# vinhsuhi/JMAC

Hardware: AMD Instinct MI355X
Metric: gnn_layer_edges_per_s (higher is better)
Workload: dtype f32

## Files before the change

include/jmac_hip.h:

```cpp
#ifndef JMAC_HIP_H_
#define JMAC_HIP_H_

#include <stddef.h>
#include <stdint.h>

#ifdef __cplusplus
extern "C" {
#endif

typedef void* jmac_stream_t;

#define JMAC_OK 0
#define JMAC_EINVAL (-1)
#define JMAC_EDIM (-2)
#define JMAC_EWORKSPACE (-3)
#define JMAC_ERANGE (-4)

typedef struct { int32_t seg, beg, end, pslot; } jmac_item_t;
typedef struct { int32_t seg, pslot0, nchunks, pad; } jmac_split_t;

const char* jmac_strerror(int rc);
int jmac_version(void);


// ... 233 lines not shown
} jmac_gemm_task_t;
int jmac_gemm_grouped_f32(const jmac_gemm_task_t* tasks, int32_t n_tasks, jmac_stream_t stream);

#define JMAC_WCAT_MAX 4
int jmac_wcat_pack_seed_f32(const float* const* w_att, const float* const* gcn, float* const* wcat, int32_t n_layers,
                            int64_t d, const float* extra_src, float* extra_dst, int64_t extra_floats,
                            int64_t* const* counters, int32_t n_counters, int64_t* seed_state, int64_t* seed_out,
                            jmac_stream_t stream);
int jmac_wcat_unpack_f32(const float* const* dwcat, float* const* d_watt, float* const* d_gcn,
                         int32_t n_layers, int64_t d, const float* extra_src, float* extra_dst,
                         int64_t extra_floats, jmac_stream_t stream);

#define JMAC_ADAM_MAX_TASKS 64
typedef struct {
    float* p;
    const float* g;
    float* m;
    float* v;
    int64_t n;
    int32_t vec4;
} jmac_adam_task_t;
int jmac_adam_step_f32(const jmac_adam_task_t* tasks, int32_t n_tasks, float* step, double* aux, double lr, double beta1,
                       double beta2, double eps, double weight_decay, int32_t decoupled, int32_t maximize, jmac_stream_t stream);

int jmac_rows_compact_f32(const float* const* h_src, const int64_t* h_ld_src, float* const* h_dst, int32_t n_tables,
                          const int64_t* idx, int64_t n_used, int64_t d, jmac_stream_t stream);
int jmac_rows_expand_f32(const float* const* h_src, float* const* h_dst, const int64_t* h_ld_dst,
                         const int32_t* h_accumulate, int32_t n_tables, const int32_t* pos, int64_t rows, int64_t d,
                         jmac_stream_t stream);


int jmac_triple_l1_fwd_f32(const float* ent, int64_t lde, const float* rel, int64_t ldr,
                           const int64_t* h, const int64_t* r, const int64_t* t, int64_t T,
                           int64_t period, int64_t d, float* score, jmac_stream_t stream);
int jmac_triple_l1_bwd_f32(const float* ent, int64_t lde, const float* rel, int64_t ldr,
                           const int64_t* h, const int64_t* r, const int64_t* t, int64_t T,
                           int64_t period, int64_t d, const float* gscore, float* dent, int64_t ldde, float* drel, int64_t lddr,
                           jmac_stream_t stream);
int jmac_pair_cosine_fwd_stats_f32(const float* e1, int64_t ld1, const float* e2, int64_t ld2, const int64_t* i1,
                                   const int64_t* i2, int64_t L, int64_t d, float* dist, float* stats,
                                   jmac_stream_t stream);
int jmac_pair_cosine_bwd_rows_f32(const float* e1, int64_t ld1, const float* e2, int64_t ld2, int64_t L, int64_t d,
                                  const float* gdist, const float* gscalar, float gscale, const float* stats,
                                  const int32_t* rec, const int32_t* rowptr, int64_t n1, int64_t n2, float* de1,
                                  int64_t ldd1, float* de2, int64_t ldd2, jmac_stream_t stream);

int jmac_triple_l1_margin_bwd_exact2_f32(const float* ent, int64_t lde, const float* rel, int64_t ldr, const int64_t* h,
                                         const int64_t* r, const int64_t* t, int64_t B, int64_t K, int64_t d,
                                         const float* score, const float* gamma, const float* gloss, int64_t ent_off,
                                         int64_t rel_off, float* cnt_ent, float* cnt_rel, float* dent, int64_t rows_ent,
                                         int32_t acc_ent, float* drel, int64_t rows_rel, int32_t acc_rel,
                                         jmac_stream_t stream);

int jmac_vec_mean_acc_f32(const float* x, int64_t n, const float* add_to, float* out, jmac_stream_t stream);

int jmac_pair_cosine_fwd_f32(const float* e1, int64_t ld1, const float* e2, int64_t ld2,
                             const int64_t* i1, const int64_t* i2, int64_t L, int64_t d, float* dist,
                             jmac_stream_t stream);
int jmac_pair_cosine_bwd_f32(const float* e1, int64_t ld1, const float* e2, int64_t ld2,
                             const int64_t* i1, const int64_t* i2, int64_t L, int64_t d,
                             const float* gdist, float* de1, int64_t ldd1, float* de2, int64_t ldd2,
                             jmac_stream_t stream);

int jmac_margin_loss_fwd_acc_f32(const float* score, int64_t B, int64_t K, const float* gamma, const float* add_to,
                                 float* loss, jmac_stream_t stream);
int jmac_margin_loss_bwd_f32(const float* score, int64_t B, int64_t K, const float* gamma,
                             const float* gloss, float* dscore, jmac_stream_t stream);


int jmac_sample_completion_batch(const int64_t* triples, int64_t T, const int64_t* perm, const int32_t* key_of_triple,
                                 const int32_t* tail_ptr, const int32_t* tail_idx, int64_t num_ent, int64_t B, int64_t K,
                                 const int64_t* seed, int64_t* step, int64_t* batch_h, int64_t* batch_r, int64_t* batch_t,
                                 jmac_stream_t stream);

int jmac_scatter_sum_f32(const float* src, const int64_t* index, int64_t E, int64_t d, int64_t N,
                         float* out, jmac_stream_t stream);
size_t jmac_scatter_softmax_workspace_bytes(int64_t N, int64_t d);
int jmac_scatter_softmax_f32(const float* src, const int64_t* index, int64_t E, int64_t d, int64_t N,
                             float* out, void* ws, size_t ws_bytes, jmac_stream_t stream);

#ifdef __cplusplus
}
#endif
#endif
```

jmac_amd/_lib.py:

```python
from __future__ import annotations

import ctypes as C
import os
import re
import weakref
from typing import Optional

_HERE = os.path.dirname(os.path.abspath(__file__))
LIB_PATH = os.environ.get("JMAC_LIB_PATH") or os.path.join(_HERE, "libjmac_hip.so")
HEADER_PATH = os.path.join(os.path.dirname(_HERE), "include", "jmac_hip.h")

_lib: Optional[C.CDLL] = None

i32, i64, f32, vp, sz = C.c_int32, C.c_int64, C.c_float, C.c_void_p, C.c_size_t


class JmacError(RuntimeError):
    pass


class View(C.Structure):
    _fields_ = [("ptr", vp), ("order", vp), ("items", vp), ("splits", vp), ("counts", vp),
                ("n_items_max", i64), ("n_splits_max", i64), ("n_parts_max", i64),
                ("item_edges", vp), ("n_empty", i64), ("n_coop", i64), ("entry_dst", vp)]
# ... 55 lines not shown
                                        vp, sz, vp]),
    "jmac_bn_tanh_bwd2_f32": (C.c_int, [vp, i64, vp, i64, vp, i64, vp, i64, i64, i64, vp, vp, vp, i32, vp, i64, vp, vp,
                                        vp, sz, vp]),
    "jmac_bn_tanh_seg_workspace_bytes": (sz, [i32, i64]),
    "jmac_bn_tanh_seg_fwd2_f32": (C.c_int, [vp, i64, i64, i32, C.POINTER(i64), C.POINTER(i32), vp, vp, vp, vp, f32, f32, vp, i64,
                                            vp, i64, vp, vp, vp, sz, vp]),
    "jmac_bn_tanh_seg_bwd2_f32": (C.c_int, [vp, i64, vp, i64, vp, i64, vp, i64, i64, i32, C.POINTER(i64), vp, vp, vp, vp, i64,
                                            vp, vp, vp, sz, vp]),
    "jmac_row_normalize_drop_fwd_f32": (C.c_int, [vp, i64, i64, i64, f32, vp, i64, f32, vp, i64, vp, vp]),
    "jmac_row_normalize_drop_bwd_f32": (C.c_int, [vp, i64, vp, vp, i64, f32, vp, i64, i64, i64, f32, vp, i64, i32, vp]),
    "jmac_row_normalize_dropseed_fwd_f32": (C.c_int, [vp, i64, i64, i64, f32, vp, f32, vp, i64, vp, vp]),
    "jmac_row_normalize_dropseed_bwd_f32": (C.c_int, [vp, i64, vp, vp, f32, vp, i64, i64, i64, f32, vp, i64, i32, vp]),
    "jmac_gemm_grouped_f32": (C.c_int, [C.POINTER(GemmTask), i32, vp]),
    "jmac_wcat_pack_seed_f32": (C.c_int, [C.POINTER(vp), C.POINTER(vp), C.POINTER(vp), i32, i64, vp, vp, i64, C.POINTER(vp), i32, vp, vp, vp]),
    "jmac_adam_step_f32": (C.c_int, [C.POINTER(AdamTask), i32, vp, vp, C.c_double, C.c_double, C.c_double, C.c_double, C.c_double, i32, i32,
                                     vp]),
    "jmac_wcat_unpack_f32": (C.c_int, [C.POINTER(vp), C.POINTER(vp), C.POINTER(vp), i32, i64, vp, vp, i64, vp]),
    "jmac_rows_compact_f32": (C.c_int, [C.POINTER(vp), C.POINTER(i64), C.POINTER(vp), i32, vp, i64, i64, vp]),
    "jmac_rows_expand_f32": (C.c_int, [C.POINTER(vp), C.POINTER(vp), C.POINTER(i64), C.POINTER(i32), i32, vp, i64, i64, vp]),
    "jmac_col_moments_f32": (C.c_int, [vp, i64, i64, i64, vp, vp, vp, sz, vp]),
    "jmac_bn_tanh_apply_f32": (C.c_int, [vp, i64, i64, i64, vp, vp, vp, vp, vp, i64, vp]),
    "jmac_bn_tanh_bwd_sums_f32": (C.c_int, [vp, i64, vp, i64, vp, i64, i64, i64, vp, vp, vp, vp, sz, vp]),
    "jmac_bn_tanh_bwd_apply_f32": (C.c_int, [vp, i64, vp, i64, vp, i64, i64, i64, vp, vp, vp, vp, i64, vp, i64, vp]),
    "jmac_row_normalize_fwd_f32": (C.c_int, [vp, i64, i64, i64, f32, vp, i64, vp, vp]),
    "jmac_row_normalize_bwd_f32": (C.c_int, [vp, i64, vp, i64, vp, i64, i64, f32, vp, i64, vp]),
    "jmac_l1_score_f32": (C.c_int, [vp, i64, vp, i64, i64, i64, i64, vp, i64, i32, vp]),
    "jmac_l1_score_bf16": (C.c_int, [vp, i64, vp, i64, i64, i64, i64, vp, i64, i32, vp]),
    "jmac_filtered_rank_f32": (C.c_int, [vp, i64, vp, vp, vp, i64, i64, i32, vp, vp]),
    "jmac_linkpred_rank_workspace_bytes": (sz, [i64, i64, i32]),
    "jmac_linkpred_rank_f32": (C.c_int, [vp, i32, vp, vp, i32, vp, vp, vp, i64, i64, i64, vp, vp, sz, vp]),
    "jmac_linkpred_rank_bf16": (C.c_int, [vp, i32, vp, vp, i32, vp, vp, vp, i64, i64, i64, vp, vp, sz, vp]),
    "jmac_sim_matrix_f32": (C.c_int, [vp, i64, vp, i64, i64, i64, i64, vp, i64, vp]),
    "jmac_sim_topk_workspace_bytes": (sz, [i64, i64, i32]),
    "jmac_sim_topk_f32": (C.c_int, [vp, i64, vp, i64, i64, i64, i64, i32, vp, vp, vp, sz, vp]),
    "jmac_col_topk_workspace_bytes": (sz, [i64, i64, i32]),
    "jmac_col_topk_f32": (C.c_int, [vp, i64, i64, i64, i32, vp, vp, sz, vp]),
    "jmac_row_topk_f32": (C.c_int, [vp, i64, i64, i64, i32, vp, vp, vp]),
    "jmac_softmax_entropy_workspace_bytes": (sz, [i64, i64]),
    "jmac_softmax_entropy_f32": (C.c_int, [vp, i64, vp, i64, i64, i64, i64, f32, vp, vp, vp, sz, vp]),
    "jmac_row_softmax_f32": (C.c_int, [vp, i64, i64, i64, vp, vp, f32, f32, vp, i64, vp, vp]),
    "jmac_col_softmax_workspace_bytes": (sz, [i64, i64]),
    "jmac_col_softmax_f32": (C.c_int, [vp, i64, i64, i64, vp, vp, f32, f32, vp, i64, vp, vp, sz, vp]),
    "jmac_csls_rank_f32": (C.c_int, [vp, i64, i64, i64, vp, vp, vp, vp, vp]),
    "jmac_csls_apply_f32": (C.c_int, [vp, i64, i64, i64, vp, vp, vp, i64, vp]),
    "jmac_gemm_f32": (C.c_int, [vp, i64, i32, vp, i64, i32, i64, i64, i64, vp, i64, vp]),
    "jmac_triple_l1_fwd_f32": (C.c_int, [vp, i64, vp, i64, vp, vp, vp, i64, i64, i64, vp, vp]),
    "jmac_triple_l1_bwd_f32": (C.c_int, [vp, i64, vp, i64, vp, vp, vp, i64, i64, i64, vp, vp, i64, vp, i64, vp]),
    "jmac_pair_cosine_fwd_stats_f32": (C.c_int, [vp, i64, vp, i64, vp, vp, i64, i64, vp, vp, vp]),
    "jmac_pair_cosine_fwd_f32": (C.c_int, [vp, i64, vp, i64, vp, vp, i64, i64, vp, vp]),
    "jmac_pair_cosine_bwd_f32": (C.c_int, [vp, i64, vp, i64, vp, vp, i64, i64, vp, vp, i64, vp, i64, vp]),
    "jmac_pair_cosine_bwd_rows_f32": (C.c_int, [vp, i64, vp, i64, i64, i64, vp, vp, f32, vp, vp, vp, i64, i64, vp, i64, vp, i64, vp]),
    "jmac_triple_l1_margin_bwd_exact2_f32": (C.c_int, [vp, i64, vp, i64, vp, vp, vp, i64, i64, i64, vp, vp, vp, i64, i64, vp, vp,
                                                       vp, i64, i32, vp, i64, i32, vp]),
    "jmac_vec_mean_acc_f32": (C.c_int, [vp, i64, vp, vp, vp]),
    "jmac_margin_loss_fwd_acc_f32": (C.c_int, [vp, i64, i64, vp, vp, vp, vp]),
    "jmac_margin_loss_bwd_f32": (C.c_int, [vp, i64, i64, vp, vp, vp, vp]),
    "jmac_sample_completion_batch": (C.c_int, [vp, i64, vp, vp, vp, vp, i64, i64, i64, vp, vp, vp, vp, vp, vp]),
    "jmac_scatter_sum_f32": (C.c_int, [vp, vp, i64, i64, i64, vp, vp]),
    "jmac_scatter_softmax_workspace_bytes": (sz, [i64, i64]),
    "jmac_scatter_softmax_f32": (C.c_int, [vp, vp, i64, i64, i64, vp, vp, sz, vp]),
}


_TESTING_SIGS = {
    "jmac_gemm_nt_x3_f32": (C.c_int, [vp, i64, vp, i64, i64, i64, i64, vp, i64, vp]),
}


def header_text(path: str = HEADER_PATH) -> str:
    return re.sub(r"/\*.*?\*/", "", open(path).read(), flags=re.S)


def header_symbols(path: str = HEADER_PATH):
    return sorted(set(re.findall(r"\b(jmac_[a-z0-9_]+)\s*\(", header_text(path))))


def lib() -> C.CDLL:
    global _lib
    if _lib is None:
        if not os.path.exists(LIB_PATH):
            raise JmacError(
                "jmac_amd: %s is missing. Build it with `python -c \"import __graft_entry__ as g; g.build()\"` "
                "(or `make -C jmac_amd/csrc`). There is no CPU fallback." % LIB_PATH)
        import torch
        l = C.CDLL(LIB_PATH)
        for name, (res, args) in _SIGS.items():
            fn = getattr(l, name)
            fn.restype = res
            fn.argtypes = args
        _lib = l
    return _lib


_tlib: Optional[C.CDLL] = None


def testing_lib() -> C.CDLL:
    global _tlib
    if _tlib is None:
        path = os.path.join(_HERE, "libjmac_hip_testing.so")
        if not os.path.exists(path):
            raise JmacError("jmac_amd: %s is missing (the atomic backward lives in the testing build only: "
                            "`make -C jmac_amd/csrc`)" % path)
        import torch
        l = C.CDLL(path)
        for name in ("jmac_rel_attn_aggregate_bwd_f32", "jmac_rel_attn_bwd_workspace_bytes", "jmac_strerror"):
# ... 88 lines not shown
```

jmac_amd/csrc/loss.hip:

```cpp
#include "common.h"

using namespace jmac;

namespace {

constexpr int kBlock = 256;
constexpr int kWavesPerBlock = kBlock / 64;

__device__ __forceinline__ float sgn(float x) { return x > 0.f ? 1.f : (x < 0.f ? -1.f : 0.f); }

template <int NK>
__global__ __launch_bounds__(kBlock) void triple_l1_fwd_kernel(const float* __restrict__ ent, int64_t lde,
                                                               const float* __restrict__ rel, int64_t ldr,
                                                               const int64_t* __restrict__ h, const int64_t* __restrict__ r,
                                                               const int64_t* __restrict__ t, int64_t T, int64_t period, int parts,
                                                               int d, float* __restrict__ score) {
    const int lane = lane_id();
    const int64_t w0 = (int64_t)blockIdx.x * kWavesPerBlock + (threadIdx.x >> 6);
    const int64_t nw = (int64_t)gridDim.x * kWavesPerBlock;
    const int64_t nrun = (period < T ? period : T) * parts;
    const int64_t stride = period * parts;
    for (int64_t u = w0; u < nrun; u += nw) {
        const int64_t b = u / parts, p = u % parts;
        int64_t ch = -1, cr = -1;
// ... 95 lines not shown
                const int c = lane + 64 * k;
                if (c < d && acc[k] != 0.f) {
                    atomicAdd(qh + c, acc[k]);
                    atomicAdd(qr + c, acc[k]);
                }
            }
        };
        int64_t x = b + p * period;
        while (x < T) {
            const int64_t x2 = x + stride;
            const bool in2 = x2 < T;
            const int64_t ih = h[x], ir = r[x], it = t[x];
            const int64_t ih2 = h[in2 ? x2 : x], ir2 = r[in2 ? x2 : x], it2 = t[in2 ? x2 : x];
            const bool pair = in2 && ih2 == ih && ir2 == ir;
            if (ih != ch || ir != cr) {
                flush();
                ch = ih;
                cr = ir;
                const float* ph = ent + ih * lde;
                const float* pr = rel + ir * ldr;
#pragma unroll
                for (int k = 0; k < NK; ++k) {
                    const int c = lane + 64 * k;
                    hr[k] = c < d ? ph[c] + pr[c] : 0.f;
                    acc[k] = 0.f;
                }
            }
            const float g = gof(x), g2 = pair ? gof(x2) : 0.f;
            const float* pt = ent + it * lde;
            const float* pt2 = ent + (pair ? it2 : it) * lde;
            float* qt = dent + it * ldde;
            float* qt2 = dent + (pair ? it2 : it) * ldde;
            float tv[NK], tv2[NK];
#pragma unroll
            for (int k = 0; k < NK; ++k) {
                const int c = lane + 64 * k;
                tv[k] = c < d ? pt[c] : 0.f;
                tv2[k] = c < d ? pt2[c] : 0.f;
            }
#pragma unroll
            for (int k = 0; k < NK; ++k) {
                const int c = lane + 64 * k;
                if (c < d) {
                    const float v = g * sgn(hr[k] - tv[k]);
                    const float v2 = g2 * sgn(hr[k] - tv2[k]);
                    acc[k] += v + v2;
                    if (v != 0.f) atomicAdd(qt + c, -v);
                    if (v2 != 0.f) atomicAdd(qt2 + c, -v2);
                }
            }
            x += pair ? 2 * stride : stride;
        }
        flush();
    }
}

constexpr float kNormEps = 1e-12f;

template <bool VEC>
__device__ __forceinline__ void pair_dots(const float* __restrict__ pa, const float* __restrict__ pb, int d, int lane,
                                          float& ab, float& aa, float& bb) {
    float s_ab = 0.f, s_aa = 0.f, s_bb = 0.f;
    if (VEC) {
        const int D4 = d >> 2;
#pragma unroll 2
        for (int c = lane; c < D4; c += 64) {
            const float4 a = ld4(pa + 4 * c), b = ld4(pb + 4 * c);
            s_ab += a.x * b.x + a.y * b.y + a.z * b.z + a.w * b.w;
            s_aa += a.x * a.x + a.y * a.y + a.z * a.z + a.w * a.w;
            s_bb += b.x * b.x + b.y * b.y + b.z * b.z + b.w * b.w;
        }
    } else {
        for (int c = lane; c < d; c += 64) {
            const float a = pa[c], b = pb[c];
            s_ab += a * b;
            s_aa += a * a;
            s_bb += b * b;
        }
    }
    float v[3] = {s_ab, s_aa, s_bb};
    wave_sum_n<3>(v);
    ab = v[0];
    aa = v[1];
    bb = v[2];
}

template <bool VEC>
__global__ __launch_bounds__(kBlock) void pair_cosine_fwd_kernel(const float* __restrict__ e1, int64_t ld1,
                                                                 const float* __restrict__ e2, int64_t ld2,
                                                                 const int64_t* __restrict__ i1, const int64_t* __restrict__ i2,
                                                                 int64_t L, int d, float* __restrict__ dist, float* __restrict__ stats) {
    const int lane = lane_id();
    const int64_t w0 = (int64_t)blockIdx.x * kWavesPerBlock + (threadIdx.x >> 6);
    const int64_t nw = (int64_t)gridDim.x * kWavesPerBlock;
    for (int64_t x = w0; x < L; x += nw) {
        float ab, aa, bb;
        pair_dots<VEC>(e1 + i1[x] * ld1, e2 + i2[x] * ld2, d, lane, ab, aa, bb);
        const float na = fmaxf(sqrtf(aa), kNormEps), nb = fmaxf(sqrtf(bb), kNormEps);
        if (lane == 0) {
            dist[x] = 1.f - ab / (na * nb);
            if (stats) *reinterpret_cast<float4*>(stats + 4 * x) = make_float4(ab, aa, bb, 0.f);
        }
    }
}

template <bool VEC>
// ... 58 lines not shown
                ow[k] = c < d ? own[c] : 0.f;
            }
            for (int q = p0; q < p1; ++q) {
                const int4 nx = rec[q + 1 < p1 ? q + 1 : q];
                const bool side = ((unsigned)rc.w & kRecSide) != 0;
                const float* partner = side ? e1 + (int64_t)rc.z * ld1 : e2 + (int64_t)rc.z * ld2;
                const float4 st = *reinterpret_cast<const float4*>(stats + 4 * (int64_t)rc.x);
                const float g = -(gscalar ? gs : gdist[rc.x]);
                float pr[NKM];
#pragma unroll
                for (int k = 0; k < NKM; ++k) {
                    const int c = lane + 64 * k;
                    pr[k] = c < d ? partner[c] : 0.f;
                }
                const float ra = sqrtf(st.y), rb = sqrtf(st.z);
                const float na = fmaxf(ra, kNormEps), nb = fmaxf(rb, kNormEps);
                const float inv = 1.f / (na * nb);
                const float c_ = st.x * inv;
                const float kself = side ? (rb > kNormEps ? c_ / (nb * nb) : 0.f) : (ra > kNormEps ? c_ / (na * na) : 0.f);
#pragma unroll
                for (int k = 0; k < NKM; ++k) acc[k] += g * (pr[k] * inv - kself * ow[k]);
                rc = nx;
            }
        }
#pragma unroll
        for (int k = 0; k < NKM; ++k) {
            const int c = lane + 64 * k;
            if (c < d) dst[c] = acc[k];
        }
    }
}

__global__ __launch_bounds__(kBlock) void scale_clear_flat2_kernel(float4* __restrict__ cnt_a, float4* __restrict__ out_a, int64_t na4,
                                                                   float4* __restrict__ cnt_b, float4* __restrict__ out_b, int64_t nb4,
                                                                   const float* __restrict__ gloss, float inv_2bk, int acc_a, int acc_b) {
    const float u = gloss[0] * inv_2bk;
    const int64_t total = na4 + nb4;
    for (int64_t i = (int64_t)blockIdx.x * kBlock + threadIdx.x; i < total; i += (int64_t)gridDim.x * kBlock) {
        const bool in_a = i < na4;
        float4* pc = in_a ? cnt_a + i : cnt_b + (i - na4);
        float4* po = in_a ? out_a + i : out_b + (i - na4);
        const float4 c = *pc;
        float4 v = make_float4(c.x * u, c.y * u, c.z * u, c.w * u);
        if (in_a ? acc_a : acc_b) {
            const float4 o = *po;
            v.x = __fadd_rn(__fmul_rn(c.x, u), o.x); v.y = __fadd_rn(__fmul_rn(c.y, u), o.y);
            v.z = __fadd_rn(__fmul_rn(c.z, u), o.z); v.w = __fadd_rn(__fmul_rn(c.w, u), o.w);
        }
        *po = v;
        if (c.x != 0.f || c.y != 0.f || c.z != 0.f || c.w != 0.f) *pc = make_float4(0.f, 0.f, 0.f, 0.f);
    }
}

inline unsigned wave_grid(int64_t units) {
    int64_t b = (units + kWavesPerBlock - 1) / kWavesPerBlock;
    if (b < 1) b = 1;
    return (unsigned)(b < 8192 ? b : 8192);
}

inline int run_parts(int64_t T, int64_t period) {
    const int64_t len = (T + period - 1) / period;
    int64_t p = (8192 + period - 1) / period;
    if (p > len) p = len;
    if (p < 1) p = 1;
    return (int)p;
}

inline bool vec_ok(int64_t d, std::initializer_list<int64_t> lds, std::initializer_list<const void*> ptrs) {
    if (d % 4) return false;
    for (int64_t l : lds)
        if (l % 4) return false;
    for (const void* p : ptrs)
        if ((uintptr_t)p % 16) return false;
    return true;
}

constexpr int kMarginBlock = 1024;
__global__ __launch_bounds__(kMarginBlock) void margin_loss_fwd_kernel(const float* __restrict__ score, int B, int K,
                                                                        const float* __restrict__ gamma_p, const float* __restrict__ add_to,
                                                                        float* __restrict__ loss) {
    __shared__ float red[kMarginBlock];
    const float gamma = gamma_p[0];
    float acc = 0.f;
    const int total = B * K;
    int i = threadIdx.x;
    for (; i + 7 * kMarginBlock < total; i += 8 * kMarginBlock) {
        float p[8], n[8];
#pragma unroll
        for (int u = 0; u < 8; ++u) {
            const int j = i + u * kMarginBlock;
            p[u] = score[(unsigned)j % (unsigned)B];
            n[u] = score[B + j];
        }
#pragma unroll
        for (int u = 0; u < 8; ++u) acc += fmaxf(p[u] - n[u], -gamma);
    }
    for (; i < total; i += kMarginBlock) acc += fmaxf(score[(unsigned)i % (unsigned)B] - score[B + i], -gamma);
    red[threadIdx.x] = acc;
    __syncthreads();
    for (int s = kMarginBlock / 2; s > 0; s >>= 1) {
        if ((int)threadIdx.x < s) red[threadIdx.x] += red[threadIdx.x + s];
        __syncthreads();
    }
    if (threadIdx.x == 0) loss[0] = (red[0] / (float)total + gamma) + (add_to ? add_to[0] : 0.f);
}

// ... 136 lines not shown
        hipLaunchKernelGGL(pair_cosine_bwd_kernel<false>, dim3(wave_grid(L)), dim3(kBlock), 0, st, e1, ld1, e2, ld2, i1, i2, L, (int)d,
                           gdist, de1, ldd1, de2, ldd2);
    return (int)hipGetLastError();
}

int jmac_margin_loss_fwd_acc_f32(const float* score, int64_t B, int64_t K, const float* gamma, const float* add_to, float* loss,
                                 jmac_stream_t stream) {
    if (B <= 0 || K <= 0 || B >= INT32_MAX || K >= INT32_MAX || B * K + B >= INT32_MAX) return JMAC_EINVAL;
    if (!score || !gamma || !loss) return JMAC_EINVAL;
    hipLaunchKernelGGL(margin_loss_fwd_kernel, dim3(1), dim3(kMarginBlock), 0, (hipStream_t)stream, score, (int)B, (int)K, gamma, add_to,
                       loss);
    return (int)hipGetLastError();
}

int jmac_vec_mean_acc_f32(const float* x, int64_t n, const float* add_to, float* out, jmac_stream_t stream) {
    if (n <= 0 || !x || !out) return JMAC_EINVAL;
    hipLaunchKernelGGL(vec_mean_acc_kernel, dim3(1), dim3(kMarginBlock), 0, (hipStream_t)stream, x, n, add_to, out);
    return (int)hipGetLastError();
}

int jmac_pair_cosine_bwd_rows_f32(const float* e1, int64_t ld1, const float* e2, int64_t ld2, int64_t L, int64_t d, const float* gdist,
                                  const float* gscalar, float gscale, const float* stats, const int32_t* rec, const int32_t* rowptr,
                                  int64_t n1, int64_t n2, float* de1, int64_t ldd1, float* de2, int64_t ldd2, jmac_stream_t stream) {
    if (L < 0 || d <= 0 || n1 < 0 || n2 < 0) return JMAC_EINVAL;
    if (d > 512) return JMAC_EDIM;
    if (n1 + n2 == 0) return JMAC_OK;
    if (2 * L >= INT32_MAX) return JMAC_ERANGE;
    if (!e1 || !e2 || (!gdist && !gscalar) || !rowptr || !de1 || (n2 > 0 && !de2)) return JMAC_EINVAL;
    if (L > 0 && (!stats || !rec || ((uintptr_t)rec & 15) || ((uintptr_t)stats & 15))) return JMAC_EINVAL;
    hipLaunchKernelGGL(pair_cosine_bwd_rows_kernel, dim3(wave_grid(n1 + n2)), dim3(kBlock), 0, (hipStream_t)stream, e1, ld1, e2, ld2, (int)d,
                       gdist, gscalar, gscale, stats, reinterpret_cast<const int4*>(rec), rowptr, n1, n2, de1, ldd1, de2 ? de2 : de1, ldd2);
    return (int)hipGetLastError();
}

int jmac_triple_l1_margin_bwd_exact2_f32(const float* ent, int64_t lde, const float* rel, int64_t ldr, const int64_t* h, const int64_t* r,
                                         const int64_t* t, int64_t B, int64_t K, int64_t d, const float* score, const float* gamma,
                                         const float* gloss, int64_t ent_off, int64_t rel_off, float* cnt_ent, float* cnt_rel,
                                         float* dent, int64_t rows_ent, int32_t acc_ent, float* drel, int64_t rows_rel, int32_t acc_rel,
                                         jmac_stream_t stream) {
    if (B <= 0 || K <= 0 || d <= 0 || B >= INT32_MAX || K >= INT32_MAX || rows_ent <= 0 || rows_rel <= 0 || ent_off < 0 || rel_off < 0 ||
        ent_off >= rows_ent || rel_off >= rows_rel)
        return JMAC_EINVAL;
    if (d > 512 || d % 4) return JMAC_EDIM;
    if (!ent || !rel || !h || !r || !t || !score || !gamma || !gloss || !cnt_ent || !cnt_rel || !dent || !drel) return JMAC_EINVAL;
    if ((((uintptr_t)cnt_ent | (uintptr_t)cnt_rel | (uintptr_t)dent | (uintptr_t)drel) & 15) != 0) return JMAC_EINVAL;
    if (4 * B * K >= (1LL << 24)) return JMAC_ERANGE;
    const int64_t T = B * (K + 1), period = B;
    hipStream_t st = (hipStream_t)stream;
    const int nk = (int)((d + 63) / 64);
    const int parts = run_parts(T, period);
    JMAC_DISPATCH_NK(nk, hipLaunchKernelGGL((triple_l1_bwd_kernel<NK, true>), dim3(wave_grid(period * parts)), dim3(kBlock), 0, st,
                                            ent, lde, rel, ldr, h, r, t, T, period, parts, (int)d, score, cnt_ent + ent_off * d, d,
                                            cnt_rel + rel_off * d, d, MarginArgs{gamma, B, K}));
    const int64_t na4 = rows_ent * d / 4, nb4 = rows_rel * d / 4;
    int64_t blocks = (na4 + nb4 + kBlock - 1) / kBlock;
    if (blocks > 4096) blocks = 4096;
    hipLaunchKernelGGL(scale_clear_flat2_kernel, dim3((unsigned)blocks), dim3(kBlock), 0, st, reinterpret_cast<float4*>(cnt_ent),
                       reinterpret_cast<float4*>(dent), na4, reinterpret_cast<float4*>(cnt_rel), reinterpret_cast<float4*>(drel), nb4, gloss,
                       1.f / (2.f * (float)B * (float)K), (int)acc_ent, (int)acc_rel);
    return (int)hipGetLastError();
}

int jmac_margin_loss_bwd_f32(const float* score, int64_t B, int64_t K, const float* gamma, const float* gloss, float* dscore,
                             jmac_stream_t stream) {
    if (B <= 0 || K <= 0 || B >= INT32_MAX || K >= INT32_MAX) return JMAC_EINVAL;
    if (!score || !gamma || !gloss || !dscore) return JMAC_EINVAL;
    hipLaunchKernelGGL(margin_loss_bwd_kernel, dim3((unsigned)((B + kBlock - 1) / kBlock)), dim3(kBlock), 0, (hipStream_t)stream, score,
                       (int)B, (int)K, gamma, gloss, dscore);
    return (int)hipGetLastError();
}

}
```

jmac_amd/csrc/scatter.hip:

```cpp
#include "common.h"

using namespace jmac;

namespace {

__device__ __forceinline__ void atomic_max_f32(float* addr, float v) {
    if (v >= 0.f) atomicMax(reinterpret_cast<int*>(addr), __float_as_int(v));
    else atomicMin(reinterpret_cast<unsigned int*>(addr), __float_as_uint(v));
}

__global__ void scatter_sum_kernel(const float* __restrict__ src, const int64_t* __restrict__ index, int64_t E, int64_t d,
                                   int64_t N, float* __restrict__ out) {
    const int64_t total = E * d;
    for (int64_t i = (int64_t)blockIdx.x * blockDim.x + threadIdx.x; i < total; i += (int64_t)gridDim.x * blockDim.x) {
        const int64_t e = i / d, c = i % d;
        const int64_t r = index[e];
        if (r >= 0 && r < N) atomicAdd(out + r * d + c, src[i]);
    }
}

__global__ void fill_f32_kernel(float* __restrict__ p, int64_t n, float v) {
    for (int64_t i = (int64_t)blockIdx.x * blockDim.x + threadIdx.x; i < n; i += (int64_t)gridDim.x * blockDim.x) p[i] = v;
}

// ... 35 lines not shown
    int64_t g = (total + 255) / 256;
    if (g < 1) g = 1;
    return (unsigned)(g < 16384 ? g : 16384);
}

}

extern "C" {

int jmac_scatter_sum_f32(const float* src, const int64_t* index, int64_t E, int64_t d, int64_t N, float* out,
                         jmac_stream_t stream) {
    if (E < 0 || d <= 0 || N < 0) return JMAC_EINVAL;
    if (E == 0) return JMAC_OK;
    if (!src || !index || !out) return JMAC_EINVAL;
    hipLaunchKernelGGL(scatter_sum_kernel, dim3(grid_for(E * d)), dim3(256), 0, (hipStream_t)stream, src, index, E, d, N, out);
    return (int)hipGetLastError();
}

size_t jmac_scatter_softmax_workspace_bytes(int64_t N, int64_t d) {
    if (N < 0 || d < 0) return 0;
    return 2 * align_up((size_t)N * (size_t)d * 4) + 256;
}

int jmac_scatter_softmax_f32(const float* src, const int64_t* index, int64_t E, int64_t d, int64_t N, float* out, void* ws,
                             size_t ws_bytes, jmac_stream_t stream) {
    if (E < 0 || d <= 0 || N < 0) return JMAC_EINVAL;
    if (E == 0) return JMAC_OK;
    if (!src || !index || !out) return JMAC_EINVAL;
    if (!ws || ws_bytes < jmac_scatter_softmax_workspace_bytes(N, d)) return JMAC_EWORKSPACE;
    hipStream_t st = (hipStream_t)stream;
    float* mx = (float*)ws;
    float* sum = (float*)((char*)ws + align_up((size_t)N * (size_t)d * 4));
    hipLaunchKernelGGL(fill_f32_kernel, dim3(grid_for(N * d)), dim3(256), 0, st, mx, N * d, -INFINITY);
    hipLaunchKernelGGL(fill_f32_kernel, dim3(grid_for(N * d)), dim3(256), 0, st, sum, N * d, 0.f);
    hipLaunchKernelGGL(seg_max_kernel, dim3(grid_for(E * d)), dim3(256), 0, st, src, index, E, d, N, mx);
    hipLaunchKernelGGL(seg_expsum_kernel, dim3(grid_for(E * d)), dim3(256), 0, st, src, index, E, d, N, mx, sum, out);
    hipLaunchKernelGGL(seg_div_kernel, dim3(grid_for(E * d)), dim3(256), 0, st, index, E, d, N, sum, out);
    return (int)hipGetLastError();
}

const char* jmac_strerror(int rc) {
    switch (rc) {
        case JMAC_OK: return "ok";
        case JMAC_EINVAL: return "jmac: invalid argument (null pointer or negative size)";
        case JMAC_EDIM: return "jmac: unsupported dimension (need d % 4 == 0, d <= 512, ld % 4 == 0)";
        case JMAC_EWORKSPACE: return "jmac: workspace missing or too small";
        case JMAC_ERANGE: return "jmac: size exceeds int32 indexing";
        default: break;
    }
    if (rc > 0) return hipGetErrorString((hipError_t)rc);
    return "jmac: unknown error";
}

int jmac_version(void) { return 126; }

}
```

jmac_amd/losses.py:

```python
from __future__ import annotations

import torch

from ._lib import check, check_index_range, lib, ptr, require_device, stream


def _fresh(*grads) -> None:
    for g in grads:
        if g is not None:
            g._jmac_fresh_grad = True


def _rows(t: torch.Tensor) -> torch.Tensor:
    if t.dtype != torch.float32:
        raise TypeError("jmac_amd losses compute in fp32 (got %s)" % t.dtype)
    return t if t.stride(-1) == 1 and t.dim() == 2 else t.contiguous()


def _index(i: torch.Tensor, n: int, device, what: str = "index") -> torch.Tensor:
    check_index_range(i, n, what)
    if i.dim() != 1:
        i = i.reshape(-1)
    if i.dtype != torch.int64 or i.device != device:
        i = i.to(device=device, dtype=torch.int64)
# ... 177 lines not shown
    i1, i2 = _index(i1, n1, dev), _index(i2, n2, dev)
    if i1.numel() == 0 or e1.shape[1] > 512:
        out = _PairCosine.apply(e1, e2, i1, i2, off1, off2).mean()
        return out if add_to is None else out + add_to
    if add_to is not None:
        add_to = add_to.reshape(1)
    return _PairCosineMean.apply(e1, e2, i1, i2, off1, off2, add_to)


def pair_cosine_distance(e1: torch.Tensor, i1: torch.Tensor, e2: torch.Tensor, i2: torch.Tensor, win1=None,
                         win2=None) -> torch.Tensor:
    dev = e1.device
    off1, n1 = _win(e1, win1)
    off2, n2 = _win(e2, win2)
    return _PairCosine.apply(e1, e2, _index(i1, n1, dev), _index(i2, n2, dev), off1, off2)


class _MarginLoss(torch.autograd.Function):
    @staticmethod
    def forward(ctx, score, margin, B, K):
        require_device(score, margin)
        score = score.contiguous()
        loss = torch.empty(1, dtype=torch.float32, device=score.device)
        check(lib().jmac_margin_loss_fwd_acc_f32(ptr(score), B, K, ptr(margin), None, ptr(loss), stream()),
              "jmac_margin_loss_fwd_acc_f32")
        ctx.save_for_backward(score, margin)
        ctx.bk = (B, K)
        return loss

    @staticmethod
    def backward(ctx, g):
        score, margin = ctx.saved_tensors
        B, K = ctx.bk
        g = g.contiguous()
        dscore = torch.empty_like(score)
        check(lib().jmac_margin_loss_bwd_f32(ptr(score), B, K, ptr(margin), ptr(g), ptr(dscore), stream()), "jmac_margin_loss_bwd_f32")
        return dscore, None, None, None


def _win(table: torch.Tensor, win):
    if win is None:
        return 0, int(table.shape[0])
    off, n = int(win[0]), int(win[1])
    if off < 0 or n < 0 or off + n > table.shape[0]:
        raise ValueError("row window [%d, %d) outside a table of %d rows" % (off, off + n, table.shape[0]))
    return off, n


def _wptr(t: torch.Tensor, off: int) -> int:
    return t.data_ptr() + off * t.stride(0) * t.element_size()


_CNT: dict = {}


def _count_tables(dev, rows_e: int, rows_r: int, d: int):
    key = (str(dev), int(rows_e), int(rows_r), int(d))
    hit = _CNT.get(key)
    if hit is None:
        hit = (torch.zeros((rows_e, d), dtype=torch.float32, device=dev), torch.zeros((rows_r, d), dtype=torch.float32, device=dev))
        if not torch.cuda.is_current_stream_capturing():
            _CNT[key] = hit
    return hit


class _LayerLoss(torch.autograd.Function):

    @staticmethod
    def forward(ctx, ent, rel, h, r, t, margin, add_to, c0, c1, B, K, eoff, roff, coff0, coff1):
        require_device(ent, rel, h, r, t, margin)
        ent, rel = _rows(ent), _rows(rel)
        T, d = h.numel(), ent.shape[1]
        if rel.shape[1] != d or r.numel() != T or t.numel() != T or T != B * (K + 1) or (c0 is not None and c1.numel() != c0.numel()):
            raise ValueError("completion_layer_loss: shapes disagree")
        dev = ent.device
        score = torch.empty(T, dtype=torch.float32, device=dev)
        loss = torch.empty(1, dtype=torch.float32, device=dev)
        check(lib().jmac_triple_l1_fwd_f32(_wptr(ent, eoff), ent.stride(0), _wptr(rel, roff), rel.stride(0), ptr(h), ptr(r), ptr(t),
                                           T, B, d, ptr(score), stream()), "jmac_triple_l1_fwd_f32")
        check(lib().jmac_margin_loss_fwd_acc_f32(ptr(score), B, K, ptr(margin), ptr(add_to), ptr(loss), stream()),
              "jmac_margin_loss_fwd_acc_f32")
        stats = None
        if c0 is not None:
            L = c0.numel()
            dist = torch.empty(L, dtype=torch.float32, device=dev)
            stats = torch.empty((L, 4), dtype=torch.float32, device=dev)
            total = torch.empty(1, dtype=torch.float32, device=dev)
            check(lib().jmac_pair_cosine_fwd_stats_f32(_wptr(ent, coff0), ent.stride(0), _wptr(ent, coff1), ent.stride(0), ptr(c0), ptr(c1),
                                                       L, d, ptr(dist), ptr(stats), stream()), "jmac_pair_cosine_fwd_stats_f32")
            check(lib().jmac_vec_mean_acc_f32(ptr(dist), L, ptr(loss), ptr(total), stream()), "jmac_vec_mean_acc_f32")
            loss = total
        ctx.save_for_backward(ent, rel, h, r, t, score, margin, c0, c1, stats)
        ctx.cfg = (B, K, eoff, roff, coff0, coff1, add_to is not None)
        return loss

    @staticmethod
    def backward(ctx, g):
        ent, rel, h, r, t, score, margin, c0, c1, stats = ctx.saved_tensors
        B, K, eoff, roff, coff0, coff1, has_add = ctx.cfg
        d = ent.shape[1]
        dev = ent.device
        g = g.contiguous()
        rows_e, rows_r = int(ent.shape[0]), int(rel.shape[0])
        dent = torch.empty((rows_e, d), dtype=torch.float32, device=dev)
        drel = torch.empty((rows_r, d), dtype=torch.float32, device=dev)
        if c0 is not None:
            _pair_cosine_rows_bwd(ent, ent, c0, c1, coff0, coff1, True, stats, None, g, float(c0.numel()), de1=dent)
        cnt_e, cnt_r = _count_tables(dev, rows_e, rows_r, d)
        check(lib().jmac_triple_l1_margin_bwd_exact2_f32(_wptr(ent, eoff), ent.stride(0), _wptr(rel, roff), rel.stride(0), ptr(h), ptr(r),
                                                         ptr(t), B, K, d, ptr(score), ptr(margin), ptr(g), eoff, roff, ptr(cnt_e),
                                                         ptr(cnt_r), ptr(dent), rows_e, 1 if c0 is not None else 0, ptr(drel), rows_r, 0,
                                                         stream()), "jmac_triple_l1_margin_bwd_exact2_f32")
        _fresh(dent, drel)
        return (dent, drel, None, None, None, None, (g if has_add else None), None, None, None, None, None, None, None, None)


def completion_layer_loss(ent: torch.Tensor, rel: torch.Tensor, h: torch.Tensor, r: torch.Tensor, t: torch.Tensor, batch_size: int,
                          margin: torch.Tensor, ent_win=None, rel_win=None, links=None, add_to: torch.Tensor = None) -> torch.Tensor:
    dev = ent.device
    T, B = int(h.numel()), int(batch_size)
    eoff, en = _win(ent, ent_win)
    roff, rn = _win(rel, rel_win)
    d = ent.shape[1]
    fused = (B > 0 and T > B and (T - B) % B == 0 and margin.numel() == 1 and not margin.requires_grad and d % 4 == 0 and d <= 512
             and 4 * B * ((T - B) // B) < (1 << 24) and ent.dtype == torch.float32 and rel.dtype == torch.float32
             and (links is None or links[0].numel() > 0))
    if not fused:
        out = margin_loss(triple_l1_score(ent[eoff:eoff + en], rel[roff:roff + rn], h, r, t, period=B), B, margin)
        if links is not None and links[0].numel() > 0:
            out = out + pair_cosine_distance(ent, links[0], ent, links[1], links[2], links[3]).mean()
        return out if add_to is None else out + add_to
    c0 = c1 = None
    coff0 = coff1 = 0
    if links is not None:
        coff0, n0 = _win(ent, links[2])
        coff1, n1 = _win(ent, links[3])
        c0, c1 = _index(links[0], n0, dev), _index(links[1], n1, dev)
    if add_to is not None:
        add_to = add_to.reshape(1)
    return _LayerLoss.apply(ent, rel, _index(h, en, dev, "batch_h"), _index(r, rn, dev, "batch_r"), _index(t, en, dev, "batch_t"),
                            margin.reshape(1).to(torch.float32), add_to, c0, c1, B, (T - B) // B, eoff, roff, coff0, coff1)


def triple_l1_margin_loss(ent: torch.Tensor, rel: torch.Tensor, h: torch.Tensor, r: torch.Tensor, t: torch.Tensor,
                          batch_size: int, margin: torch.Tensor, ent_win=None, rel_win=None) -> torch.Tensor:
    return completion_layer_loss(ent, rel, h, r, t, batch_size, margin, ent_win, rel_win)


def margin_loss(score: torch.Tensor, batch_size: int, margin: torch.Tensor) -> torch.Tensor:
    T, B = int(score.numel()), int(batch_size)
    if score.dim() != 1 or score.dtype != torch.float32 or margin.numel() != 1 or margin.requires_grad \
            or T <= B or (T - B) % B != 0:
        pos, neg = score[:B], score[B:]
        pos = pos.view(-1, min(B, len(pos))).permute(1, 0)
        neg = neg.view(-1, min(B, len(neg))).permute(1, 0)
        return torch.max(pos - neg, -margin).mean() + margin
    return _MarginLoss.apply(score, margin.reshape(1).to(torch.float32), B, (T - B) // B)
```

Baseline: 29.66 million.

## Fuse margin-gradient count accumulation into forward scoring kernel with leased count tables

When gradients are needed, the forward pass now uses a one-pass kernel that computes triple L1 scores and also accumulates the margin-loss sign counts into per-row tables with atomics. It relies on each positive triple's negatives sharing head and relation to keep those rows in registers. The backward pass then only runs the scale-and-clear kernel, so it no longer re-gathers embeddings and recomputes differences. In exchange, forward carries extra atomic traffic, and a lease system keeps count tables alive between forward and backward, adding bookkeeping and the risk of dirty tables if backward never runs.

```diff
diff --git a/include/jmac_hip.h b/include/jmac_hip.h
--- a/include/jmac_hip.h
+++ b/include/jmac_hip.h
@@ -309,6 +309,14 @@
                                          int32_t acc_ent, float* drel, int64_t rows_rel, int32_t acc_rel,
                                          jmac_stream_t stream);
 
+int jmac_triple_l1_margin_fwd_counts_f32(const float* ent, int64_t lde, const float* rel, int64_t ldr, const int64_t* h,
+                                         const int64_t* r, const int64_t* t, int64_t B, int64_t K, int64_t d,
+                                         const float* gamma, int64_t ent_off, int64_t rel_off, float* cnt_ent,
+                                         float* cnt_rel, float* score, jmac_stream_t stream);
+int jmac_margin_counts_scale_clear_f32(float* cnt_ent, float* cnt_rel, const float* gloss, int64_t B, int64_t K, int64_t d,
+                                       float* dent, int64_t rows_ent, int32_t acc_ent, float* drel, int64_t rows_rel,
+                                       int32_t acc_rel, jmac_stream_t stream);
+
 int jmac_vec_mean_acc_f32(const float* x, int64_t n, const float* add_to, float* out, jmac_stream_t stream);
 
 int jmac_pair_cosine_fwd_f32(const float* e1, int64_t ld1, const float* e2, int64_t ld2,
diff --git a/jmac_amd/_lib.py b/jmac_amd/_lib.py
--- a/jmac_amd/_lib.py
+++ b/jmac_amd/_lib.py
@@ -131,6 +131,8 @@
     "jmac_pair_cosine_bwd_rows_f32": (C.c_int, [vp, i64, vp, i64, i64, i64, vp, vp, f32, vp, vp, vp, i64, i64, vp, i64, vp, i64, vp]),
     "jmac_triple_l1_margin_bwd_exact2_f32": (C.c_int, [vp, i64, vp, i64, vp, vp, vp, i64, i64, i64, vp, vp, vp, i64, i64, vp, vp,
                                                        vp, i64, i32, vp, i64, i32, vp]),
+    "jmac_triple_l1_margin_fwd_counts_f32": (C.c_int, [vp, i64, vp, i64, vp, vp, vp, i64, i64, i64, vp, i64, i64, vp, vp, vp, vp]),
+    "jmac_margin_counts_scale_clear_f32": (C.c_int, [vp, vp, vp, i64, i64, i64, vp, i64, i32, vp, i64, i32, vp]),
     "jmac_vec_mean_acc_f32": (C.c_int, [vp, i64, vp, vp, vp]),
     "jmac_margin_loss_fwd_acc_f32": (C.c_int, [vp, i64, i64, vp, vp, vp, vp]),
     "jmac_margin_loss_bwd_f32": (C.c_int, [vp, i64, i64, vp, vp, vp, vp]),
diff --git a/jmac_amd/csrc/loss.hip b/jmac_amd/csrc/loss.hip
--- a/jmac_amd/csrc/loss.hip
+++ b/jmac_amd/csrc/loss.hip
@@ -171,6 +171,162 @@
             x += pair ? 2 * stride : stride;
         }
         flush();
+    }
+}
+
+constexpr int kOnePassWaves = 4;
+__device__ __forceinline__ float margin_w2(float diff, float gamma) { return diff > -gamma ? 2.f : (diff == -gamma ? 1.f : 0.f); }
+__device__ __forceinline__ int64_t uniform(int64_t v) {
+    const uint32_t lo = __builtin_amdgcn_readfirstlane((uint32_t)v), hi = __builtin_amdgcn_readfirstlane((uint32_t)((uint64_t)v >> 32));
+    return (int64_t)(((uint64_t)hi << 32) | lo);
+}
+
+template <int NK, int NW>
+__global__ __launch_bounds__(64 * NW) void triple_l1_margin_fwd_counts_kernel(const float* __restrict__ ent, int64_t lde,
+                                                                              const float* __restrict__ rel, int64_t ldr,
+                                                                              const int64_t* __restrict__ h, const int64_t* __restrict__ r,
+                                                                              const int64_t* __restrict__ t, int B, int K, int d,
+                                                                              const float* __restrict__ gamma_p, float* __restrict__ score,
+                                                                              float* __restrict__ cnt_ent, float* __restrict__ cnt_rel) {
+    __shared__ float red[NW][NK * 64];
+    __shared__ float red_g[NW];
+    const int lane = lane_id(), wave = (int)(threadIdx.x >> 6);
+    const float gamma = gamma_p[0];
+    for (int b = blockIdx.x; b < B; b += gridDim.x) {
+        const int64_t ih = uniform(h[b]), ir = uniform(r[b]), itp = uniform(t[b]);
+        float hr[NK], tp[NK], acc[NK];
+        {
+            const float* ph = ent + ih * lde;
+            const float* pr = rel + ir * ldr;
+            const float* pt = ent + itp * lde;
+#pragma unroll
+            for (int k = 0; k < NK; ++k) {
+                const int c = lane + 64 * k;
+                hr[k] = c < d ? ph[c] + pr[c] : 0.f;
+                tp[k] = c < d ? pt[c] : 0.f;
+                acc[k] = 0.f;
+            }
+        }
+        float pos = 0.f;
+#pragma unroll
+        for (int k = 0; k < NK; ++k)
+            if (lane + 64 * k < d) pos += fabsf(hr[k] - tp[k]);
+        pos = wave_sum(pos);
+        if (wave == 0 && lane == 0) score[b] = pos;
+        float g2w = 0.f;
+        auto single = [&](int64_t x, int64_t xh, int64_t xr, int64_t xt) {
+            const bool own = xh != ih || xr != ir;
+            const float* ph = ent + xh * lde;
+            const float* pr = rel + xr * ldr;
+            const float* pt = ent + xt * lde;
+            float df[NK], s = 0.f;
+#pragma unroll
+            for (int k = 0; k < NK; ++k) {
+                const int c = lane + 64 * k;
+                const float a = own ? (c < d ? ph[c] + pr[c] : 0.f) : hr[k];
+                df[k] = a - (c < d ? pt[c] : 0.f);
+                if (c < d) s += fabsf(df[k]);
+            }
+            s = wave_sum(s);
+            if (lane == 0) score[x] = s;
+            const float w2 = margin_w2(pos - s, gamma);
+            g2w += w2;
+            float* qt = cnt_ent + xt * d;
+            float* qh = cnt_ent + xh * d;
+            float* qr = cnt_rel + xr * d;
+#pragma unroll
+            for (int k = 0; k < NK; ++k) {
+                const int c = lane + 64 * k;
+                const float v = -w2 * sgn(df[k]);
+                if (c < d && v != 0.f) {
+                    atomicAdd(qt + c, -v);
+                    if (own) {
+                        atomicAdd(qh + c, v);
+                        atomicAdd(qr + c, v);
+                    } else {
+                        acc[k] += v;
+                    }
+                }
+            }
+        };
+        for (int j = wave; j < K; j += 2 * NW) {
+            const bool in2 = j + NW < K;
+            const int64_t x = (int64_t)B + (int64_t)j * B + b;
+            const int64_t x2 = in2 ? x + (int64_t)NW * B : x;
+            const int64_t xh = uniform(h[x]), xr = uniform(r[x]), xt = uniform(t[x]);
+            const int64_t xh2 = uniform(h[x2]), xr2 = uniform(r[x2]), xt2 = uniform(t[x2]);
+            if (xh != ih || xr != ir || xh2 != ih || xr2 != ir) {
+                single(x, xh, xr, xt);
+                if (in2) single(x2, xh2, xr2, xt2);
+                continue;
+            }
+            const float* pt = ent + xt * lde;
+            const float* pt2 = ent + xt2 * lde;
+            float tv[NK], tv2[NK];
+#pragma unroll
+            for (int k = 0; k < NK; ++k) {
+                const int c = lane + 64 * k;
+                tv[k] = c < d ? pt[c] : 0.f;
+                tv2[k] = c < d ? pt2[c] : 0.f;
+            }
+            float s[2] = {0.f, 0.f};
+#pragma unroll
+            for (int k = 0; k < NK; ++k) {
+                if (lane + 64 * k < d) {
+                    s[0] += fabsf(hr[k] - tv[k]);
+                    s[1] += fabsf(hr[k] - tv2[k]);
+                }
+            }
+            wave_sum_n<2>(s);
+            if (lane == 0) {
+                score[x] = s[0];
+                if (in2) score[x2] = s[1];
+            }
+            const float w2a = margin_w2(pos - s[0], gamma);
+            const float w2b = in2 ? margin_w2(pos - s[1], gamma) : 0.f;
+            g2w += w2a + w2b;
+            float* qt = cnt_ent + xt * d;
+            float* qt2 = cnt_ent + xt2 * d;
+#pragma unroll
+            for (int k = 0; k < NK; ++k) {
+                const int c = lane + 64 * k;
+                if (c < d) {
+                    const float v = -w2a * sgn(hr[k] - tv[k]);
+                    const float v2 = -w2b * sgn(hr[k] - tv2[k]);
+                    acc[k] += v + v2;
+                    if (v != 0.f) atomicAdd(qt + c, -v);
+                    if (v2 != 0.f) atomicAdd(qt2 + c, -v2);
+                }
+            }
+        }
+#pragma unroll
+        for (int k = 0; k < NK; ++k) red[wave][lane + 64 * k] = acc[k];
+        if (lane == 0) red_g[wave] = g2w;
+        __syncthreads();
+        float G = 0.f;
+#pragma unroll
+        for (int w = 0; w < NW; ++w) G += red_g[w];
+        float* qh = cnt_ent + ih * d;
+        float* qr = cnt_rel + ir * d;
+        float* qp = cnt_ent + itp * d;
+#pragma unroll
+        for (int k = 0; k < NK; ++k) {
+            if (k % NW != wave) continue;
+            const int c = lane + 64 * k;
+            if (c < d) {
+                float tot = 0.f;
+#pragma unroll
+                for (int w = 0; w < NW; ++w) tot += red[w][c];
+                const float vp = G * sgn(hr[k] - tp[k]);
+                tot += vp;
+                if (tot != 0.f) {
+                    atomicAdd(qh + c, tot);
+                    atomicAdd(qr + c, tot);
+                }
+                if (vp != 0.f) atomicAdd(qp + c, -vp);
+            }
+        }
+        __syncthreads();
     }
 }
 
@@ -335,6 +491,16 @@
     }
 }
 
+inline void launch_scale_clear(float* cnt_ent, float* cnt_rel, const float* gloss, int64_t B, int64_t K, int64_t d, float* dent,
+                               int64_t rows_ent, int32_t acc_ent, float* drel, int64_t rows_rel, int32_t acc_rel, hipStream_t st) {
+    const int64_t na4 = rows_ent * d / 4, nb4 = rows_rel * d / 4;
+    int64_t blocks = (na4 + nb4 + kBlock - 1) / kBlock;
+    if (blocks > 4096) blocks = 4096;
+    hipLaunchKernelGGL(scale_clear_flat2_kernel, dim3((unsigned)blocks), dim3(kBlock), 0, st, reinterpret_cast<float4*>(cnt_ent),
+                       reinterpret_cast<float4*>(dent), na4, reinterpret_cast<float4*>(cnt_rel), reinterpret_cast<float4*>(drel), nb4, gloss,
+                       1.f / (2.f * (float)B * (float)K), (int)acc_ent, (int)acc_rel);
+}
+
 inline unsigned wave_grid(int64_t units) {
     int64_t b = (units + kWavesPerBlock - 1) / kWavesPerBlock;
     if (b < 1) b = 1;
@@ -577,12 +743,34 @@
     JMAC_DISPATCH_NK(nk, hipLaunchKernelGGL((triple_l1_bwd_kernel<NK, true>), dim3(wave_grid(period * parts)), dim3(kBlock), 0, st,
                                             ent, lde, rel, ldr, h, r, t, T, period, parts, (int)d, score, cnt_ent + ent_off * d, d,
                                             cnt_rel + rel_off * d, d, MarginArgs{gamma, B, K}));
-    const int64_t na4 = rows_ent * d / 4, nb4 = rows_rel * d / 4;
-    int64_t blocks = (na4 + nb4 + kBlock - 1) / kBlock;
-    if (blocks > 4096) blocks = 4096;
-    hipLaunchKernelGGL(scale_clear_flat2_kernel, dim3((unsigned)blocks), dim3(kBlock), 0, st, reinterpret_cast<float4*>(cnt_ent),
-                       reinterpret_cast<float4*>(dent), na4, reinterpret_cast<float4*>(cnt_rel), reinterpret_cast<float4*>(drel), nb4, gloss,
-                       1.f / (2.f * (float)B * (float)K), (int)acc_ent, (int)acc_rel);
+    launch_scale_clear(cnt_ent, cnt_rel, gloss, B, K, d, dent, rows_ent, acc_ent, drel, rows_rel, acc_rel, st);
+    return (int)hipGetLastError();
+}
+
+int jmac_triple_l1_margin_fwd_counts_f32(const float* ent, int64_t lde, const float* rel, int64_t ldr, const int64_t* h, const int64_t* r,
+                                         const int64_t* t, int64_t B, int64_t K, int64_t d, const float* gamma, int64_t ent_off,
+                                         int64_t rel_off, float* cnt_ent, float* cnt_rel, float* score, jmac_stream_t stream) {
+    if (B <= 0 || K <= 0 || d <= 0 || B >= INT32_MAX || K >= INT32_MAX || ent_off < 0 || rel_off < 0) return JMAC_EINVAL;
+    if (d > 512 || d % 4) return JMAC_EDIM;
+    if (!ent || !rel || !h || !r || !t || !gamma || !cnt_ent || !cnt_rel || !score) return JMAC_EINVAL;
+    if (4 * B * K >= (1LL << 24)) return JMAC_ERANGE;
+    constexpr int NW = kOnePassWaves;
+    const int nk = (int)((d + 63) / 64);
+    const unsigned grid = (unsigned)(B < 65536 ? B : 65536);
+    JMAC_DISPATCH_NK(nk, hipLaunchKernelGGL((triple_l1_margin_fwd_counts_kernel<NK, NW>), dim3(grid), dim3(64 * NW), 0, (hipStream_t)stream,
+                                            ent, lde, rel, ldr, h, r, t, (int)B, (int)K, (int)d, gamma, score, cnt_ent + ent_off * d,
+                                            cnt_rel + rel_off * d));
+    return (int)hipGetLastError();
+}
+
+int jmac_margin_counts_scale_clear_f32(float* cnt_ent, float* cnt_rel, const float* gloss, int64_t B, int64_t K, int64_t d, float* dent,
+                                       int64_t rows_ent, int32_t acc_ent, float* drel, int64_t rows_rel, int32_t acc_rel,
+                                       jmac_stream_t stream) {
+    if (B <= 0 || K <= 0 || d <= 0 || rows_ent <= 0 || rows_rel <= 0) return JMAC_EINVAL;
+    if (d % 4) return JMAC_EDIM;
+    if (!cnt_ent || !cnt_rel || !gloss || !dent || !drel) return JMAC_EINVAL;
+    if ((((uintptr_t)cnt_ent | (uintptr_t)cnt_rel | (uintptr_t)dent | (uintptr_t)drel) & 15) != 0) return JMAC_EINVAL;
+    launch_scale_clear(cnt_ent, cnt_rel, gloss, B, K, d, dent, rows_ent, acc_ent, drel, rows_rel, acc_rel, (hipStream_t)stream);
     return (int)hipGetLastError();
 }
 
diff --git a/jmac_amd/csrc/scatter.hip b/jmac_amd/csrc/scatter.hip
--- a/jmac_amd/csrc/scatter.hip
+++ b/jmac_amd/csrc/scatter.hip
@@ -111,6 +111,6 @@
     return "jmac: unknown error";
 }
 
-int jmac_version(void) { return 126; }
+int jmac_version(void) { return 127; }
 
 }
diff --git a/jmac_amd/losses.py b/jmac_amd/losses.py
--- a/jmac_amd/losses.py
+++ b/jmac_amd/losses.py
@@ -253,22 +253,61 @@
 
 
 _CNT: dict = {}
-
-
-def _count_tables(dev, rows_e: int, rows_r: int, d: int):
-    key = (str(dev), int(rows_e), int(rows_r), int(d))
-    hit = _CNT.get(key)
-    if hit is None:
-        hit = (torch.zeros((rows_e, d), dtype=torch.float32, device=dev), torch.zeros((rows_r, d), dtype=torch.float32, device=dev))
-        if not torch.cuda.is_current_stream_capturing():
-            _CNT[key] = hit
-    return hit
+_CNT_DIRTY: list = []
+_CNT_PINNED: list = []
+_CNT_SERIAL = [0]
+
+
+class _Lease:
+
+    __slots__ = ("key", "pair")
+
+    def __init__(self, key, pair):
+        self.key, self.pair = key, pair
+
+    def release(self, clean: bool, reusable: bool = True) -> None:
+        key, pair, self.pair = self.key, self.pair, None
+        if pair is None or key is None:
+            return
+        if not reusable or (key[4] and not clean):
+            _CNT_PINNED.append(pair)
+        elif clean:
+            _CNT[key] = pair
+        else:
+            _CNT_DIRTY.append((key, pair))
+
+    def __del__(self):
+        try:
+            self.release(False)
+        except Exception:
+            pass
+
+
+def _take_tables(dev, rows_e: int, rows_r: int, d: int) -> _Lease:
+    shape = (str(dev), int(rows_e), int(rows_r), int(d))
+    capturing = torch.cuda.is_current_stream_capturing()
+    for want in ((True, False) if capturing else (False,)):
+        for key in _CNT:
+            if key[:4] == shape and key[4] == want:
+                return _Lease(key[:4] + (capturing, key[5]), _CNT.pop(key))
+    if not capturing:
+        for i, (key, pair) in enumerate(_CNT_DIRTY):
+            if key[:4] == shape and not key[4]:
+                del _CNT_DIRTY[i]
+                pair[0].zero_()
+                pair[1].zero_()
+                return _Lease(key, pair)
+    pair = (torch.zeros((rows_e, d), dtype=torch.float32, device=dev), torch.zeros((rows_r, d), dtype=torch.float32, device=dev))
+    if capturing:
+        return _Lease(None, pair)
+    _CNT_SERIAL[0] += 1
+    return _Lease(shape + (False, _CNT_SERIAL[0]), pair)
 
 
 class _LayerLoss(torch.autograd.Function):
 
     @staticmethod
-    def forward(ctx, ent, rel, h, r, t, margin, add_to, c0, c1, B, K, eoff, roff, coff0, coff1):
+    def forward(ctx, ent, rel, h, r, t, margin, add_to, c0, c1, B, K, eoff, roff, coff0, coff1, counts):
         require_device(ent, rel, h, r, t, margin)
         ent, rel = _rows(ent), _rows(rel)
         T, d = h.numel(), ent.shape[1]
@@ -277,8 +316,17 @@
         dev = ent.device
         score = torch.empty(T, dtype=torch.float32, device=dev)
         loss = torch.empty(1, dtype=torch.float32, device=dev)
-        check(lib().jmac_triple_l1_fwd_f32(_wptr(ent, eoff), ent.stride(0), _wptr(rel, roff), rel.stride(0), ptr(h), ptr(r), ptr(t),
-                                           T, B, d, ptr(score), stream()), "jmac_triple_l1_fwd_f32")
+        ctx.lease = None
+        if counts:
+            lease = _take_tables(dev, int(ent.shape[0]), int(rel.shape[0]), d)
+            cnt_e, cnt_r = lease.pair
+            check(lib().jmac_triple_l1_margin_fwd_counts_f32(_wptr(ent, eoff), ent.stride(0), _wptr(rel, roff), rel.stride(0), ptr(h),
+                                                             ptr(r), ptr(t), B, K, d, ptr(margin), eoff, roff, ptr(cnt_e), ptr(cnt_r),
+                                                             ptr(score), stream()), "jmac_triple_l1_margin_fwd_counts_f32")
+            ctx.lease = lease
+        else:
+            check(lib().jmac_triple_l1_fwd_f32(_wptr(ent, eoff), ent.stride(0), _wptr(rel, roff), rel.stride(0), ptr(h), ptr(r), ptr(t),
+                                               T, B, d, ptr(score), stream()), "jmac_triple_l1_fwd_f32")
         check(lib().jmac_margin_loss_fwd_acc_f32(ptr(score), B, K, ptr(margin), ptr(add_to), ptr(loss), stream()),
               "jmac_margin_loss_fwd_acc_f32")
         stats = None
@@ -307,13 +355,24 @@
         drel = torch.empty((rows_r, d), dtype=torch.float32, device=dev)
         if c0 is not None:
             _pair_cosine_rows_bwd(ent, ent, c0, c1, coff0, coff1, True, stats, None, g, float(c0.numel()), de1=dent)
-        cnt_e, cnt_r = _count_tables(dev, rows_e, rows_r, d)
-        check(lib().jmac_triple_l1_margin_bwd_exact2_f32(_wptr(ent, eoff), ent.stride(0), _wptr(rel, roff), rel.stride(0), ptr(h), ptr(r),
-                                                         ptr(t), B, K, d, ptr(score), ptr(margin), ptr(g), eoff, roff, ptr(cnt_e),
-                                                         ptr(cnt_r), ptr(dent), rows_e, 1 if c0 is not None else 0, ptr(drel), rows_r, 0,
-                                                         stream()), "jmac_triple_l1_margin_bwd_exact2_f32")
+        lease, ctx.lease = ctx.lease, None
+        if lease is not None and lease.pair is not None:
+            cnt_e, cnt_r = lease.pair
+            same = lease.key is None or lease.key[4] == torch.cuda.is_current_stream_capturing()
+            check(lib().jmac_margin_counts_scale_clear_f32(ptr(cnt_e), ptr(cnt_r), ptr(g), B, K, d, ptr(dent), rows_e,
+                                                           1 if c0 is not None else 0, ptr(drel), rows_r, 0, stream()),
+                  "jmac_margin_counts_scale_clear_f32")
+            lease.release(True, reusable=same)
+        else:
+            lease = _take_tables(dev, rows_e, rows_r, d)
+            cnt_e, cnt_r = lease.pair
+            check(lib().jmac_triple_l1_margin_bwd_exact2_f32(_wptr(ent, eoff), ent.stride(0), _wptr(rel, roff), rel.stride(0), ptr(h),
+                                                             ptr(r), ptr(t), B, K, d, ptr(score), ptr(margin), ptr(g), eoff, roff,
+                                                             ptr(cnt_e), ptr(cnt_r), ptr(dent), rows_e, 1 if c0 is not None else 0,
+                                                             ptr(drel), rows_r, 0, stream()), "jmac_triple_l1_margin_bwd_exact2_f32")
+            lease.release(True)
         _fresh(dent, drel)
-        return (dent, drel, None, None, None, None, (g if has_add else None), None, None, None, None, None, None, None, None)
+        return (dent, drel, None, None, None, None, (g if has_add else None), None, None, None, None, None, None, None, None, None)
 
 
 def completion_layer_loss(ent: torch.Tensor, rel: torch.Tensor, h: torch.Tensor, r: torch.Tensor, t: torch.Tensor, batch_size: int,
@@ -340,7 +399,8 @@
     if add_to is not None:
         add_to = add_to.reshape(1)
     return _LayerLoss.apply(ent, rel, _index(h, en, dev, "batch_h"), _index(r, rn, dev, "batch_r"), _index(t, en, dev, "batch_t"),
-                            margin.reshape(1).to(torch.float32), add_to, c0, c1, B, (T - B) // B, eoff, roff, coff0, coff1)
+                            margin.reshape(1).to(torch.float32), add_to, c0, c1, B, (T - B) // B, eoff, roff, coff0, coff1,
+                            torch.is_grad_enabled() and (ent.requires_grad or rel.requires_grad))
 
 
 def triple_l1_margin_loss(ent: torch.Tensor, rel: torch.Tensor, h: torch.Tensor, r: torch.Tensor, t: torch.Tensor,
```

New measurement: 31.01 million, median of 6. +4.6%, better.
